# motionlife/gqmap-opticalflow

Measured on AMD Instinct MI355X. Metric: Gpixel-iters/s + AEPE vs .flo GT, Middlebury 584x388, 1/2/4/8 GPU, higher is better.
Workload: dtype f64; 1 GPU; C2: rubberwhale 584x388 mixture L=1 K=9 its=2541 (one step = one full-frame iteration); engine=mixture, L=1, K=9, parallelism=frame-parallel x1

## Files before the change

gqmap-opticalflow_amd/csrc/gqmap_engine.hip:

```cpp
#include <dlfcn.h>
#include <hip/hip_runtime.h>
#include <rccl/rccl.h>

#include <algorithm>
#include <chrono>
#include <condition_variable>
#include <cstdlib>
#include <cmath>
#include <cstring>
#include <mutex>
#include <string>
#include <vector>

#include "gqmap_internal.h"
#include "gqmap_blockmatch.h"

#pragma clang fp contract(off)

namespace gq {
__device__ __forceinline__ double gq_sqrt_dev(double x)
{
    const double y = __builtin_amdgcn_rsq(x);
    double g = x * y, h = 0.5 * y;
    const double r = fma(-h, g, 0.5);
// ... 67 lines not shown
    }
    __device__ __forceinline__ float end() const { return rp > 0.f ? sp : r; }
};
}
#define GQ_ROOT_STAGED 1

#define GQ_HD __device__ __forceinline__
#define GQ_SQRT(x) gq::gq_sqrt_dev(x)
#include "gqmap_tuning.h"
#define GQ_STR2(x) #x
#define GQ_PRAGMA_UNROLL(n) _Pragma(GQ_STR2(unroll n))
#define GQ_UNROLL2 GQ_PRAGMA_UNROLL(GQ_EDGE_UNROLL_N)
#define GQ_PAIR_UNROLL GQ_PRAGMA_UNROLL(GQ_PAIR_UNROLL_N)
#define GQ_PAIR_UNROLL_K(n) GQ_PRAGMA_UNROLL(n)
#define GQ_NODE_UNROLL GQ_PRAGMA_UNROLL(GQ_NODE_UNROLL_N)
#define GQ_UNROLL_FULL _Pragma("unroll")
#define GQ_UMUL24(a, b) __umul24((uint32_t)(a), (uint32_t)(b))
#define GQ_FRACT(x) __builtin_amdgcn_fract(x)
#define GQ_LDS_AS __attribute__((address_space(3)))
#define GQ_LUT_AT(lut, o) (*(const GQ_LDS_AS double *)((const GQ_LDS_AS char *)(lut) + (o)))
#define GQ_SCHED_FENCE __builtin_amdgcn_sched_barrier(0)
#define GQ_PIN64(x) asm volatile("" : "+v"(x))
#define GQ_PIN_UNIFORM(x) asm volatile("" : "+s"(x))
#include "gqmap_math.h"

namespace gq {

typedef float vvs_t;

constexpr int TILE = 16;
constexpr int BLOCK = TILE * TILE;
constexpr int TS = TAB_STRIDE;
constexpr int NPLANES = 9;
constexpr int TRACE_CAP = 8192;
constexpr int GRAPH_CHUNK = 50;
#ifndef GQ_FLOW_CHUNK
#define GQ_FLOW_CHUNK 250
#endif
constexpr int FLOW_CHUNK = GQ_FLOW_CHUNK;
static_assert(FLOW_CHUNK >= 1 && FLOW_CHUNK <= TRACE_CAP, "a launch's trace rows fit the ring");
constexpr int NFIX = 5;
constexpr int ACC_SLICES = 8;
constexpr int TRACE_W = 4;

struct Ctl {
    int it;
    int done;
    int stop;
    int arrive;
    double T;
    double alpha[GQMAP_LMAX];
    double w[GQMAP_LMAX];
    unsigned long long acc[ACC_SLICES][NFIX + GQMAP_LMAX][4];
    alignas(128) int it_i;
    int done_i;
    double T_i;
// ... 49 lines not shown
};

template <typename R>
using ctab_t = const __attribute__((address_space(4))) R *;
template <typename R>
__device__ __forceinline__ ctab_t<R> as_const(const R *p)
{
    return (ctab_t<R>)p;
}

__device__ __forceinline__ fix128 shfl_xor_fix(fix128 v, int o)
{
    const int64_t hi = (int64_t)(v >> 64);
    const uint64_t lo = (uint64_t)v;
    const int64_t h2 = __shfl_xor(hi, o, 64);
    const uint64_t l2 = (uint64_t)__shfl_xor((int64_t)lo, o, 64);
    return ((fix128)h2 << 64) | (fix128)l2;
}
__device__ __forceinline__ fix128 wave_sum_fix(fix128 v)
{
#pragma unroll
    for (int o = 32; o > 0; o >>= 1) v += shfl_xor_fix(v, o);
    return v;
}
__device__ __forceinline__ int wave_sum_small(int v)
{
    int s = 0;
#pragma unroll
    for (int b = 0; b < 6; ++b) s += __popcll(__ballot((v >> b) & 1)) << b;
    return s;
}
__device__ __forceinline__ bool finite_d(double x) { return (bits_of(x) & 0x7ff0000000000000ULL) != 0x7ff0000000000000ULL; }

__device__ __forceinline__ double shfl_xor_r(double v, int o) { return __shfl_xor(v, o, 64); }
__device__ __forceinline__ float shfl_xor_r(float v, int o) { return __shfl_xor(v, o, 64); }

typedef float f2v __attribute__((ext_vector_type(2)));

__device__ __forceinline__ f2v pk_fma(f2v a, f2v b, f2v c) { return __builtin_elementwise_fma(a, b, c); }

__device__ __forceinline__ f2v sqrt2_pk(f2v x)
{
    const f2v s = {__builtin_amdgcn_sqrtf(x.x), __builtin_amdgcn_sqrtf(x.y)};
    const f2v sm = {__int_as_float(__float_as_int(s.x) - 1), __int_as_float(__float_as_int(s.y) - 1)};
    const f2v sp = {__int_as_float(__float_as_int(s.x) + 1), __int_as_float(__float_as_int(s.y) + 1)};
    const f2v rm = pk_fma(-sm, s, x), rp = pk_fma(-sp, s, x);
// ... 296 lines not shown
           nn + P.n_off <= P.Ng - 2;
}

template <bool COH, typename R>
__device__ __forceinline__ R ld_state(const R *p)
{
    if constexpr (COH) return __hip_atomic_load(p, __ATOMIC_RELAXED, __HIP_MEMORY_SCOPE_AGENT);
    else return *p;
}
template <bool COH, typename R, bool NT = false>
__device__ __forceinline__ void st_state(R *p, R v)
{
    if constexpr (COH) __hip_atomic_store(p, v, __ATOMIC_RELAXED, __HIP_MEMORY_SCOPE_AGENT);
    else if constexpr (NT) __builtin_nontemporal_store(v, p);
    else *p = v;
}

template <typename R>
struct EdgeJob {
    int dir, uv, hr;
    bool need;
    R u1, o1, p, o2, u2;
};
template <typename R, typename VT, int Q, int TM, int TN, bool COH>
__device__ __forceinline__ EdgeJob<R> edge_job(const IterParams<R, VT> &P, const R *__restrict__ src, int e,
                                               int tid, int m, int n, int m0, int n0, int64_t loff, bool inner,
                                               bool valid, R mu_u, R mu_v, R sg_u, R sg_v)
{
    EdgeJob<R> jb{};
    int hm, hn, rm, rn;
    const bool own_edge = e < 4;
    if (own_edge) {
        jb.dir = e & 1; jb.uv = e >> 1;
        hm = m; hn = n;
        rm = jb.dir == 0 ? m + 1 : m; rn = jb.dir == 1 ? n + 1 : n;
    } else {
        const int h = tid / Q;
        const bool top = h < 2 * TN;
        const int hh = top ? h : h - 2 * TN, span = top ? TN : TM;
        jb.uv = hh / span;
        jb.hr = hh % span;
        jb.dir = top ? 0 : 1;
        hm = top ? m0 - 1 : m0 + jb.hr; hn = top ? n0 + jb.hr : n0 - 1;
        rm = top ? m0 : hm;             rn = top ? hn : n0;
    }
    const int M = P.M, N = P.N;
    const int64_t MNL = P.MNL;
    const bool r_inner = rm < M && rn < N && node_interior(P, rm, rn);
    jb.need = own_edge ? (inner || (valid && r_inner)) : (hm >= 0 && hn >= 0 && r_inner);
    if (jb.need) {
        const int uv = jb.uv;
        const int64_t h = hm + (int64_t)M * hn + loff;
        const int64_t r = rm + (int64_t)M * rn + loff;
        jb.u1 = own_edge ? (uv ? mu_v : mu_u) : ld_state<COH>(src + h + MNL * uv);
        jb.o1 = own_edge ? (uv ? sg_v : sg_u) : ld_state<COH>(src + h + MNL * (2 + uv));
        jb.p = ld_state<COH>(src + h + MNL * (5 + jb.dir + 2 * uv));
        jb.o2 = ld_state<COH>(src + r + MNL * (2 + uv));
        jb.u2 = ld_state<COH>(src + r + MNL * uv);
    }
    return jb;
}

#ifndef GQ_FLOW_TL
#define GQ_FLOW_TL 0
#endif

template <typename R>
struct HaloChain {
    R s[6][64];
    unsigned flag[4];
    unsigned *fail;
};
// ... 100 lines not shown
    __shared__ unsigned long long sh[4 * (NFIX + GQMAP_LMAX)];
    if (tid < 4 * NP) {
        unsigned long long *a = &ctl->acc[0][0][0] + tid;
        unsigned long long v[ACC_SLICES];
#pragma unroll
        for (int x = 0; x < ACC_SLICES; ++x) v[x] = __hip_atomic_load(a + x * SL, __ATOMIC_RELAXED, __HIP_MEMORY_SCOPE_AGENT);
        unsigned long long t = 0;
#pragma unroll
        for (int x = 0; x < ACC_SLICES; ++x) t += v[x];
#pragma unroll
        for (int x = 0; x < ACC_SLICES; ++x) __hip_atomic_store(a + x * SL, 0ull, __ATOMIC_RELAXED, __HIP_MEMORY_SCOPE_AGENT);
        sh[tid] = t;
    }
    __syncthreads();
    if (tid < NP) {
        fix128 v = 0;
#pragma unroll
        for (int k = 3; k >= 0; --k) v = (v << 32) + (fix128)(long long)sh[4 * tid + k];
        out[tid] = v;
    }
    if (tid == 0) ctl->arrive = 0;
}

template <typename R, typename VT>
__device__ __forceinline__ auto tile_frame_view(const IterParams<R, VT> &P, const GQ_LDS_AS double *taplut)
{
    if constexpr (is_vvo2<VT>::value) {
        return frame_view_lut(P.VV, P.M2, taplut);
    } else {
        (void)taplut;
        return frame_view(P.VV, P.M2);
    }
}

template <typename R, typename VT, int ENG, int Q, bool EDGE_FIRST, bool COH = false, bool NT = false,
          bool LIT = false, bool GRP = false, int ROTF = GQ_NODE_ROT_OTHER, int HALO = 0>
__device__ __forceinline__ void iter_tile(const IterParams<R, VT> P, int tile, int it, int parity,
                                          int part_r, TileLdsQ<R, Q> &lds, int l0, int l1, double Tcur,
                                          bool tab_ready, unsigned long long *acc_ring = nullptr,
                                          int grows = 0, bool grouped = false, HaloChain<R> *hc = nullptr,
                                          unsigned halo_tok = 0, const GQ_LDS_AS double *taplut = nullptr
#if GQ_FLOW_TL
                                          , unsigned long long *tlw = nullptr
#endif
                                          )
{
    static_assert(HALO == 0 || (GRP && sizeof(R) == 8), "the halo forms: the fp64 dataflow item (one component per item)");
    constexpr bool CHAIN = HALO == 1;
    static_assert(!LIT || (ENG == 0 && Q == 1 && sizeof(R) == 8), "literal order: fp64 mixture, Q = 1");
    static_assert(!GRP || (Q == 1 && !LIT), "a tile per wave: one lane per node");
    constexpr bool RS = Q == 0;
    constexpr int QA = arith_q(Q);
    constexpr int TPIX = tile_pix(Q);
    constexpr int TM = tile_rows(Q), TN = TPIX / TM;
    static_assert(TM * TN == TPIX, "tile");
    Ctl *ctl = P.ctl;
    const R *__restrict__ src = parity ? P.st1 : P.st0;
    R *__restrict__ dst = parity ? P.st0 : P.st1;
    const R T = R(Tcur);
    const R step = R(P.step0 / (1.0 + it / P.step_decay));

    const int tm = tile % P.tiles_m, tn = tile / P.tiles_m;
    const int tid = threadIdx.x;
    const int rtid = RS ? tid % TPIX : tid;
    const bool do_node = !RS || tid < TPIX, do_edge = !RS || tid >= TPIX;
    const int pix = rtid / QA, kj = rtid % QA;
    int lm = pix % TM, ln = pix / TM;
    if constexpr (GRP) {
        lm = (tid & 63) % grows;
        ln = (grouped ? 0 : (tid >> 6) * (64 / TM)) + (tid & 63) / grows;
    }
// ... 43 lines not shown
        const int64_t i = m + (int64_t)M * n + MN * l;
        const R mu_u = valid ? ld_state<COH>(src + i) : R(0);
        const R mu_v = valid ? ld_state<COH>(src + i + MNL) : R(0);
        const R sg_u = valid ? ld_state<COH>(src + i + MNL * 2) : R(0);
        const R sg_v = valid ? ld_state<COH>(src + i + MNL * 3) : R(0);
        const R pn = valid ? ld_state<COH>(src + i + MNL * 4) : R(0);
        Grad<R> nd{};
        R sum_mu0 = 0, sum_mu1 = 0, sum_sg0 = 0, sum_sg1 = 0;
        R eE = 0, eda = 0;
#pragma unroll
        for (int ph = 0; ph < 2; ++ph) {
        if ((ph == 0) != EDGE_FIRST) {
        if (do_node && LIT) {
            if constexpr (LIT)
                if (inner)
                    nd = lit_node_grad(tab, K2, P.VV, P.M2, P.I1, P.Mo, P.No, P.epsn, P.lamd, P.guard != 0, T, a,
                                       mu_u, mu_v, sg_u, sg_v, pn, m, n + P.n_off);
        } else if (do_node) {
        NodeCoef<R> c{};
        if (inner) c = node_coef(sg_u, sg_v, pn);
        const bool fast = ENG == 0 && __all(!inner || node_unclamped(c, mu_u, mu_v, m, n + P.n_off, P.Mo, P.No,
                                                                     P.gh_xmax, R(ENG == 2 ? CTF_MARGIN : 0.0)));
        if (inner) {
            const auto fv = tile_frame_view(P, taplut);
            constexpr bool PF = QA >= GQ_NODE_PF_MIN_Q && (QA > 1 || sizeof(VT) == 4);
            constexpr int ROT = PF ? ROTF : 0;
            Sums<R> S = fast ? node_sums<ENG, false, PF, ROT>(tab, kj, K2, QA, fv, P.I1, P.Mo, P.No, P.epsn, c, mu_u,
                                                              mu_v, m, n + P.n_off)
                             : node_sums<ENG, true, PF, ROT>(tab, kj, K2, QA, fv, P.I1, P.Mo, P.No, P.epsn, c, mu_u,
                                                             mu_v, m, n + P.n_off);
            if (QA > 1) S = lane_combine<QA>(S);
            nd = node_epi(S, c, P.lamd, P.guard != 0, T, a, sg_u, sg_v, pn, ENG == 2);
            if constexpr (RS) {
                lds.nd[0][pix] = nd.du1; lds.nd[1][pix] = nd.du2; lds.nd[2][pix] = nd.do1;
                lds.nd[3][pix] = nd.do2; lds.nd[4][pix] = nd.dp; lds.nd[5][pix] = nd.E; lds.nd[6][pix] = nd.da;
            }
        }
        }
        } else if (do_edge) {
        static_assert(HALO_LANES % QA == 0, "a node's lanes share their job count");
        const int njobs = halo_lane || chain ? 5 : 4;
        constexpr bool PREFETCH = QA >= GQ_PREFETCH_MIN_Q;
        auto job_at = [&](int e) {
            return edge_job<R, VT, QA, TM, TN, COH>(P, src, e, htid, m, n, m0, n0, MN * l, inner, valid, mu_u, mu_v,
                                                sg_u, sg_v);
        };
        EdgeJob<R> next{};
        if (PREFETCH) next = job_at(0);
        constexpr bool JOBS_UNROLLED = QA >= GQ_UNROLL_MIN_Q && ENG != 1;
        constexpr int JOB_UNROLL = JOBS_UNROLLED ? 5 : 1;
        static_assert(!CHAIN || (!PREFETCH && !JOBS_UNROLLED), "the chain: one job body, streamed");
#pragma unroll JOB_UNROLL
        for (int st = 0; st < (JOBS_UNROLLED ? 5 : njobs); ++st) {
            if (JOBS_UNROLLED && st >= njobs) continue;
            int e = st;
            bool slice = false, last = true;
            if constexpr (CHAIN)
                if (chain) {
                    slice = st == cw;
                    e = slice ? 4 : st - (st > cw);
                    last = !slice || cw == 3;
                }
            EdgeJob<R> jb;
            if (PREFETCH) {
                jb = next;
                if (st + 1 < njobs) next = job_at(st + 1);
            } else {
                jb = job_at(e);
// ... 34 lines not shown
                    g = edge_epi(S, c, P.lams, P.guard != 0, T, a, jb.o1, jb.o2, jb.p, ENG == 2);
                    }
                }
                if (own_edge && inner && lead)
                    st_state<COH, R, NT>(dst + i + MNL * (5 + e), fmin(fmax(jb.p + g.dp * step, -P.corr), P.corr));
            }
            if (own_edge) {
                if (uv == 0) { sum_mu0 = sum_mu0 + g.du1; sum_sg0 = sum_sg0 + g.do1; }
                else         { sum_mu1 = sum_mu1 + g.du1; sum_sg1 = sum_sg1 + g.do1; }
                eE = eE + g.E;
                eda = eda + g.da;
                if constexpr (GRP) {
                    if (dir == 0 && lm + 1 < grows && ln < TN) { in_up[uv][0][pix + 1] = g.du2; in_up[uv][1][pix + 1] = g.do2; }
                    if (dir == 1 && ln + 1 < TN) { in_left[uv][0][pix + grows] = g.du2; in_left[uv][1][pix + grows] = g.do2; }
                } else {
                if (lead && dir == 0 && lm + 1 < TM) { in_up[uv][0][pix + 1] = g.du2; in_up[uv][1][pix + 1] = g.do2; }
                if (lead && dir == 1 && ln + 1 < TN) { in_left[uv][0][pix + TM] = g.du2; in_left[uv][1][pix + TM] = g.do2; }
                }
            } else if constexpr (GRP) {
                const int hb = grouped ? wave * 64 : 0;
                if (CHAIN && !last) {
                    if constexpr (CHAIN) halo_chain_pass(hc, halo_tok, cw, lane, hs);
                } else
                if (dir == 0) { in_up[uv][0][hb + hr * grows] = g.du2; in_up[uv][1][hb + hr * grows] = g.do2; }
                else if (hr < grows) { in_left[uv][0][hb + hr] = g.du2; in_left[uv][1][hb + hr] = g.do2; }
            } else if (rtid % QA == 0) {
                if (dir == 0) { in_up[uv][0][hr * TM] = g.du2; in_up[uv][1][hr * TM] = g.do2; }
                else          { in_left[uv][0][hr] = g.du2; in_left[uv][1][hr] = g.do2; }
            }
#if GQ_FLOW_TL
            if (tlw && lane == 0 && own_edge) tlw[4 * cw + 1] = __builtin_amdgcn_s_memrealtime();
#endif
        }
        }
        if (ph == 0) TL_STAMP(1, __builtin_amdgcn_s_memrealtime());
        }
#if GQ_FLOW_TL
        if (tlw && lane == 0) {
            tlw[4 * cw] = (unsigned)__builtin_amdgcn_s_getreg((31 << 11) | 4);
            tlw[4 * cw + 2] = __builtin_amdgcn_s_memrealtime();
        }
#endif
        __syncthreads();
        TL_STAMP(2, __builtin_amdgcn_s_memrealtime());
        fix128 fda = 0;
        if (inner && lead && do_edge) {
            if constexpr (RS) {
                nd.du1 = lds.nd[0][pix]; nd.du2 = lds.nd[1][pix]; nd.do1 = lds.nd[2][pix];
                nd.do2 = lds.nd[3][pix]; nd.dp = lds.nd[4][pix]; nd.E = lds.nd[5][pix]; nd.da = lds.nd[6][pix];
            }
            const R gmu_u = ((nd.du1 + sum_mu0) + in_up[0][0][pix]) + in_left[0][0][pix];
            const R gmu_v = ((nd.du2 + sum_mu1) + in_up[1][0][pix]) + in_left[1][0][pix];
            const R gsg_u = ((nd.do1 + sum_sg0) + in_up[0][1][pix]) + in_left[0][1][pix];
            const R gsg_v = ((nd.do2 + sum_sg1) + in_up[1][1][pix]) + in_left[1][1][pix];
            fda = node_apply<ENG, COH, NT>(P, dst, i, m, n, step, mu_u, mu_v, sg_u, sg_v, pn, nd, gmu_u, gmu_v, gsg_u, gsg_v,
                                  eE, eda, fE, fmu, fsg, fae, nonfinite);
        }
        if (P.L > 1) {
            fda = wave_sum_fix(fda);
            if (lane == 0) red[NFIX + l][wave] = fda;
        }
        __syncthreads();
    }

    TL_STAMP(3, __builtin_amdgcn_s_memrealtime());
    fE = wave_sum_fix(fE);
    fmu = wave_sum_fix(fmu);
    fsg = wave_sum_fix(fsg);
    const fix128 fnf = (fix128)wave_sum_small(nonfinite);
    if (ENG == 2) fae = wave_sum_fix(fae);
    if (lane == 0) {
        red[0][wave] = fE;
        red[1][wave] = fmu;
        red[2][wave] = fsg;
        red[3][wave] = fnf;
        red[4][wave] = fae;
    }
    __syncthreads();
    const int NP = NFIX + P.L;
    if (tid < NP) {
        fix128 v = 0;
        const int lq = tid - NFIX;
        if (tid < NFIX || (P.L > 1 && lq >= l0 && lq < l1))
            v = (red[tid][0] + red[tid][1]) + (red[tid][2] + red[tid][3]);
        if (acc_ring) {
            if (v != 0) acc_add_agent(acc_ring + ((blockIdx.x % ACC_SLICES) * (NFIX + GQMAP_LMAX) + tid) * 4, v);
        } else if (P.fused || P.tile_acc) {
            if (v != 0) acc_add_agent(&ctl->acc[blockIdx.x % ACC_SLICES][tid][0], v);
        } else {
            store_part_agent(P.partials, P.fin.nblocks, part_r, tid, v);
        }
    }
}


template <typename R, typename VT, int ENG, int Q, bool NT = false, bool LIT = false>
__device__ __forceinline__ void k_iter_body(const IterParams<R, VT> &P)
{
    Ctl *ctl = P.ctl;
// ... 521 lines not shown
template <typename R, typename VT, int ENG, int Q, bool LIT = false, int W = 0>
__global__ __launch_bounds__(BLOCK, W > 0 ? W : LIT ? GQ_FLOW_LIT_WAVES : Q == 1 ? GQ_FLOW_WAVES : ENG == 1 ? 2 : min_waves(ENG, Q))
void k_iter_flow(IterParams<R, VT> P, int n_iter, unsigned *fl, int ntiles, const Ctl *snap)
{
    static_assert(Q >= 1 && Q <= 4, "1..4 lanes per node");
    static_assert(!LIT || (ENG == 0 && Q == 1), "literal order: the mixture engine at one lane per node");
    unsigned *bar = P.bar;
    const bool run = !snap->stop && __hip_atomic_load(&P.ctl->stop, __ATOMIC_RELAXED, __HIP_MEMORY_SCOPE_AGENT) == 0 &&
                     __hip_atomic_load(bar + BAR_FAIL, __ATOMIC_RELAXED, __HIP_MEMORY_SCOPE_AGENT) == 0;
    const int it0 = snap->it, done0 = snap->done;
    const double T0 = snap->T;
    const int b = blockIdx.x, xcd = b & 7;
    int s0 = 0;
    for (int y = 0; y < xcd; ++y) s0 += (ntiles - y + 7) >> 3;
    const int nb = (ntiles - xcd + 7) >> 3;
    const int L = ENG == 1 ? P.L : 1, nitems = ntiles * L;
    constexpr bool GRP = GQ_FLOW_GROUPS && Q == 1 && !LIT && (ENG == 0 || ENG == 2);
    constexpr int ROTF = ENG == 0 && Q == 1 && !LIT && W == 0 && sizeof(R) == 8 && is_vvpair<VT>::value
                             ? ((is_vvo2<VT>::value ? 0 : GQ_NODE_ROT_FLOW_FP64) | NODE_UNROLL(GQ_NODE_UNROLL_FLOW_FP64))
                             : GQ_NODE_ROT_OTHER;
    constexpr int HALO = !GRP || LIT || W != 0 || sizeof(R) != 8 ? 0
                         : ENG == 0 && is_vvpair<VT>::value ? GQ_FLOW_HALO
                         : ENG == 2 ? GQ_FLOW_HALO_CTF : 0;
    HaloChain<R> *hc = nullptr;
    if constexpr (HALO == 1) {
        __shared__ HaloChain<R> sh_halo;
        hc = &sh_halo;
        if (threadIdx.x < 4) sh_halo.flag[threadIdx.x] = 0;
        if (threadIdx.x == 0) sh_halo.fail = bar + BAR_FAIL;
    }
    const GQ_LDS_AS double *taplut = nullptr;
    if constexpr (is_vvo2<VT>::value) {
        __shared__ double sh_taplut[TAPLUT_N];
        const int *hdr = reinterpret_cast<const int *>(P.VV + vv_elems(P.Mo, P.No));
        const int vmin = hdr[0], vn = min(hdr[1], TAPLUT_N);
        for (int e = threadIdx.x; e < vn; e += BLOCK) sh_taplut[e] = taplut_entry(e, vmin);
        taplut = (const GQ_LDS_AS double *)sh_taplut;
    }
    const int vr = P.M - (P.tiles_m - 1) * tile_rows(Q);
    const bool groups = GRP && GQ_FLOW_ROWS && vr <= 4;
    const int nlast = groups ? (s0 + nb) / P.tiles_m - s0 / P.tiles_m : 0;
    const int nbl = groups ? nb - nlast + ((nlast + 3) >> 2) : nb * L;
    constexpr int INV = ENG == 2 && Q == 1 ? GQ_PHASE_MIX_CTF_Q1_INV : GQ_PHASE_MIX_OTHER_INV;
    constexpr bool MIX = GQ_FLOW_MIX && ENG == 0 && (!LIT || GQ_FLOW_LIT_MIX);
    const bool edge_first = MIX && ((((b >> 3) / P.cu_slots) & 1) != INV);
    __shared__ TileLdsQ<R, Q> lds;
// ... 43 lines not shown
        if (GQ_FLOW_LAG > 2 && threadIdx.x == 0)
            __hip_atomic_fetch_max(fl + FL_MAXJ, (unsigned)(j + 1), __ATOMIC_RELAXED, __HIP_MEMORY_SCOPE_AGENT);
#if GQ_FLOW_TL
        const unsigned long long tl_go = __builtin_amdgcn_s_memrealtime();
#endif
        double T = T0;
        if (P.fin.t_decay_every > 0) {
            const int e = P.fin.t_decay_every;
            const int nd = (it + e - 1) / e - (it0 + e - 1) / e;
            for (int q = 0; q < nd; ++q) T = fmax(T * P.fin.drate, P.fin.t_min);
        }
        unsigned long long *slot = acc + (size_t)(j % FL_SLOTS) * FL_ACC_SLOT;
        const int l0 = ENG == 1 ? l : 0, l1 = ENG == 1 ? l + 1 : 1;
        const int wtile = GRP ? __builtin_amdgcn_readfirstlane(grouped ? sh_grp[threadIdx.x >> 6] : tile) : tile;
        const int wrows = grouped ? vr : tile_rows(Q);
#if GQ_FLOW_TL
        const size_t tlwi = (size_t)j * nitems + (size_t)tile * L + l;
        unsigned long long *tlw = (tlwi + 1) * 16 <= (size_t)(4 * FLOW_TL_WORDS) && snap->it == 1 ? g_flow_tlw + tlwi * 16 : nullptr;
#define GQ_TLW_ARG , tlw
#else
#define GQ_TLW_ARG
#endif
        if (MIX && edge_first)
            iter_tile<R, VT, ENG, Q, true, GQ_FLOW_COH, false, LIT, GRP, ROTF, HALO>(P, wtile, it, parity, 0, lds, l0, l1, T, false, slot,
                                                                                wrows, grouped, hc, (unsigned)i + 1, taplut GQ_TLW_ARG);
        else
            iter_tile<R, VT, ENG, Q, false, GQ_FLOW_COH, false, LIT, GRP, ROTF, HALO>(P, wtile, it, parity, 0, lds, l0, l1, T, false, slot,
                                                                                 wrows, grouped, hc, (unsigned)i + 1, taplut GQ_TLW_ARG);
#undef GQ_TLW_ARG
        asm volatile("s_waitcnt vmcnt(0)" ::: "memory");
        __syncthreads();
#if GQ_FLOW_TL
        const size_t tli = (size_t)j * nitems + (size_t)tile * L + l;
        if (threadIdx.x == 0 && (tli + 1) * 4 <= (size_t)FLOW_TL_WORDS && snap->it == 1) {
            unsigned long long *w = g_flow_tl + tli * 4;
            w[0] = tl_claim;
            w[1] = tl_go;
            w[2] = __builtin_amdgcn_s_memrealtime();
            w[3] = ((unsigned long long)__builtin_amdgcn_s_getreg((31 << 11) | 20) << 32) |
                   (unsigned)__builtin_amdgcn_s_getreg((31 << 11) | 4);
        }
#endif
        if (GRP && grouped && threadIdx.x > 0 && (int)threadIdx.x < gsize)
            __hip_atomic_store(fl + FL_DONE + sh_grp[threadIdx.x], (unsigned)(j + 1), __ATOMIC_RELAXED, __HIP_MEMORY_SCOPE_AGENT);
        if (threadIdx.x == 0) {
            __hip_atomic_store(fl + FL_DONE + tile * L + l, (unsigned)(j + 1), __ATOMIC_RELAXED, __HIP_MEMORY_SCOPE_AGENT);
            const unsigned tk = __hip_atomic_fetch_add(fl + FL_ARR + (j % FL_SLOTS) * FL_LINE, (unsigned)gsize, __ATOMIC_RELAXED,
                                                       __HIP_MEMORY_SCOPE_AGENT);
            if (GQ_FLOW_PAIR) sh_i = (int)__hip_atomic_fetch_add(q, 1u, __ATOMIC_RELAXED, __HIP_MEMORY_SCOPE_AGENT);
            sh_last = tk == (unsigned)(nitems - gsize);
// ... 1248 lines not shown
    }
    if (c->lit) return false;
    if constexpr (sizeof(R) == 8) {
        switch (c->kq) {
        case 1: return launch_flow_q<R, VT, 2, 1>(c, n, dry);
        case 2: return launch_flow_q<R, VT, 2, 2>(c, n, dry);
        case 4: return c->pol.flow > 0 && launch_flow_q<R, VT, 2, 4>(c, n, dry);
        default: return false;
        }
    }
    return false;
}

bool launch_flow(gqmap_ctx *c, int n, bool dry)
{
    const bool on = c->pol.flow > 0 || (c->pol.flow < 0 && !c->fp32);
    if (!on || c->persist_off || (c->L != 1 && c->opt.engine != GQMAP_ENGINE_SUPER) || c->n_tiles != 1 ||
        c->comm || c->nranks != 0 || !fused_finalize(c) || n < 1)
        return false;
    if (c->fp32)
        return c->vvp ? !c->lit && c->kq == 1 && launch_flow_q<float, vvh2_t, 0, 1>(c, n, dry)
                      : launch_flow_t<float, float>(c, n, dry);
#if GQ_TAP_LUT
    if (c->vvp && c->tapt && c->tiles_m * c->tiles_n <= GQ_FLOW_WIDE_ITEMS)
        return !c->lit && c->kq == 1 && launch_flow_q<double, vvo2_t, 0, 1>(c, n, dry);
#endif
    if (c->vvp) return !c->lit && c->kq == 1 && launch_flow_q<double, vvh2_t, 0, 1>(c, n, dry);
    if (c->vv32) return launch_flow_t<double, vvs_t>(c, n, dry);
    return launch_flow_t<double, double>(c, n, dry);
}

gqmap_status persist_recover(gqmap_ctx *c, bool *recovered)
{
    *recovered = false;
    if (!c->d_snap) return GQMAP_OK;
    c->ctl_known = false;
    unsigned f = 0;
    GQ_HIP(hipMemcpyAsync(&f, c->d_bar + BAR_FAIL, sizeof(f), hipMemcpyDeviceToHost, c->stream));
    GQ_HIP(hipStreamSynchronize(c->stream));
    if (f == 0) return GQMAP_OK;
    Ctl h;
    GQ_HIP(hipMemcpyAsync(&h, c->d_snap_ctl, sizeof(Ctl), hipMemcpyDeviceToHost, c->stream));
    GQ_HIP(hipStreamSynchronize(c->stream));
    GQ_HIP(hipMemcpyAsync(c->d_st[h.done & 1], c->d_snap, c->snap_bytes, hipMemcpyDeviceToDevice, c->stream));
    GQ_HIP(hipMemcpyAsync(c->d_ctl, c->d_snap_ctl, sizeof(Ctl), hipMemcpyDeviceToDevice, c->stream));
    GQ_HIP(hipMemsetAsync(c->d_bar, 0, sizeof(unsigned) * BAR_WORDS, c->stream));
    if (c->d_flow) GQ_HIP(hipMemsetAsync(c->d_flow, 0, sizeof(unsigned) * c->flow_n, c->stream));
// ... 1498 lines not shown
```

gqmap-opticalflow_amd/csrc/gqmap_math.h:

```cpp
#pragma once
#include <stdint.h>
#include <string.h>

#include <type_traits>

namespace gq {

#ifndef GQ_M_PI
#define GQ_M_PI 3.14159265358979323846
#define GQ_M_SQRT2 1.41421356237309504880
#endif

constexpr int TAB_STRIDE = 256;
constexpr int NTAB = 8;
constexpr int T_XI = 0, T_XJ = 1, T_W = 2, T_WA = 3, T_WXI = 4, T_WXJ = 5, T_WM = 6, T_WX = 7;
#ifdef __HIPCC__
__host__ __device__
#endif
constexpr int tab_at(int r, int k) { return k * NTAB + r; }

GQ_HD uint64_t bits_of(double x)
{
    uint64_t u;
    memcpy(&u, &x, 8);
// ... 100 lines not shown
    w0 = fma(t2, R(2) - t, -t);
    w1 = fma(-t2, b, R(2) - t2);
    w2 = fma(t2, b, t);
    w3 = fma(t2, t, -t2);
}

#ifndef GQ_FRACT
#define GQ_FRACT(x) ((x) - floor(x))
#endif

#ifndef GQ_UMUL24
#define GQ_UMUL24(a, b) ((uint32_t)(a) * (uint32_t)(b))
#endif

template <typename VP>
GQ_HD VP byte_ptr(VP VV, uint32_t bytes)
{
    return (VP)((const char *)VV + bytes);
}
template <typename VP>
GQ_HD VP elem_ptr(VP VV, uint32_t elem)
{
    return byte_ptr(VV, elem * (uint32_t)sizeof(*VV));
}

#if defined(__HIPCC__)
struct alignas(4) vvh2_t {
    _Float16 lo, hi;
};
template <typename T>
struct is_vvh2 : std::is_same<typename std::remove_cv<T>::type, vvh2_t> {};
#else
template <typename T>
struct is_vvh2 : std::false_type {};
#endif
constexpr int TAPLUT_N = 1276;
struct alignas(4) vvo2_t {
    uint16_t lo, hi;
};
template <typename T>
struct is_vvo2 : std::is_same<typename std::remove_cv<T>::type, vvo2_t> {};
template <typename T>
struct is_vvpair : std::integral_constant<bool, is_vvh2<T>::value || is_vvo2<T>::value> {};
#ifdef __HIPCC__
__host__ __device__
#endif
// ... 136 lines not shown

template <typename VP>
struct TapView {
    VP p;
    uint32_t ld;
    GQ_HD uint32_t cell(int iy, int ix) const { return cell_elem(iy, ix, (int)ld); }
};
template <typename VP>
GQ_HD TapView<VP> frame_view(VP VV, int M2)
{
    return TapView<VP>{VV, (uint32_t)M2};
}
template <typename VP, typename LP>
struct TapViewLut {
    VP p;
    uint32_t ld;
    LP lut;
    GQ_HD uint32_t cell(int iy, int ix) const { return cell_elem(iy, ix, (int)ld); }
};
template <typename VP, typename LP>
GQ_HD TapViewLut<VP, LP> frame_view_lut(VP VV, int M2, LP lut)
{
    return TapViewLut<VP, LP>{VV, (uint32_t)M2, lut};
}
template <typename LP>
GQ_HD Taps16<double> lut_taps16(LP lut, const Taps16<vvo2_t> &T, uint32_t mask = 0xffffu, uint32_t shift = 16)
{
    Taps16<double> D;
    for (int c = 0; c < 4; ++c)
        for (int r = 0; r < 4; ++r) {
            const vvo2_t &e = T.v[4 * (c >> 1) + r];
            const uint32_t w = (uint32_t)e.lo | (uint32_t)e.hi << 16;
            D.v[4 * c + r] = GQ_LUT_AT(lut, (c & 1) ? w >> shift : w & mask);
        }
    return D;
}

constexpr int VV_TAIL = 8;
constexpr size_t vv_elems(int Mo, int No) { return (size_t)(Mo + 2) * (size_t)(No + 3) + VV_TAIL; }

template <bool CLAMP = true>
GQ_HD void axis_cell_abs(double X, int n, int &ix, double &fr)
{
    if (CLAMP) X = fmin(fmax(X, 1.0), (double)n);
    ix = (int)X;
    fr = GQ_FRACT(X);
// ... 373 lines not shown

template <typename R>
struct NodeCoef {
    R s, t, ax, bx, ay, by;
};
template <typename R>
GQ_HD NodeCoef<R> node_coef(R o1, R o2, R p)
{
    NodeCoef<R> c;
    spectral_st(p, c.s, c.t);
    const R sq2 = R(GQ_M_SQRT2);
    c.ax = sq2 * o1 * c.s; c.bx = sq2 * o1 * c.t;
    c.ay = sq2 * o2 * c.t; c.by = sq2 * o2 * c.s;
    return c;
}
constexpr int NODE_ROT = 1, NODE_ROT_STAGE = 2, NODE_ROT_FLAGS = 255;
constexpr int NODE_UNROLL(int n) { return n << 8; }
constexpr int node_rot_unroll(int rot) { return (rot >> 8) > 1 ? (rot >> 8) : 1; }
#ifndef GQ_SCHED_FENCE
#define GQ_SCHED_FENCE (void)0
#define GQ_PIN64(x) (void)(x)
#define GQ_PIN_UNIFORM(x) (void)(x)
#endif
template <bool CLAMP, int UNR, typename TP, typename TV, typename IP>
GQ_HD Sums<double> node_sums_lut(TP tab, int k0, int K2, int dk, const TV &V, IP I1, int Mo, int No, double eps,
                                 const NodeCoef<double> &c, double u1, double u2, int m, int n)
{
    Sums<double> S;
    if (k0 >= K2) return S;
    const double I = I1[m + (int64_t)Mo * n];
    const double U1 = u1 + double(n + 1), U2 = u2 + double(m + 1);
    auto locate = [&](double xi, double xj, double &so, double &to) -> uint32_t {
        const double x1 = fma(c.ax, xi, fma(c.bx, xj, U1));
        const double x2 = fma(c.ay, xi, fma(c.by, xj, U2));
        return cell4_abs_v<CLAMP>(V, Mo, No, x1, x2, so, to);
    };
    const int klast = k0 + (K2 - 1 - k0) / dk * dk;
    double so, to;
    auto T = load_taps16(V.p, locate(tab[tab_at(T_XI, k0)], tab[tab_at(T_XJ, k0)], so, to), V.ld);
    const int kn0 = k0 + dk <= klast ? k0 + dk : klast;
    double nxi = tab[tab_at(T_XI, kn0)], nxj = tab[tab_at(T_XJ, kn0)];
    auto trip = [&](int k) {
        uint32_t mask = 0xffffu, shift = 16;
        GQ_PIN_UNIFORM(mask);
        GQ_PIN_UNIFORM(shift);
        const Taps16<double> D = lut_taps16(V.lut, T, mask, shift);
        GQ_SCHED_FENCE;
        double sok = so, tok = to;
        T = load_taps16(V.p, locate(nxi, nxj, so, to), V.ld);
        GQ_SCHED_FENCE;
        GQ_PIN64(sok);
        GQ_PIN64(tok);
        const int kn2 = k + 2 * dk <= klast ? k + 2 * dk : klast;
        nxi = tab[tab_at(T_XI, kn2)];
        nxj = tab[tab_at(T_XJ, kn2)];
        const double d = fma(bicubic_taps4<double>(D, sok, tok), -0.25, I);
        S.add(tab, k, GQ_SQRT(fma(d, d, eps)));
        GQ_PIN64(S.s0); GQ_PIN64(S.sxi); GQ_PIN64(S.sxj);
        GQ_PIN64(S.sa); GQ_PIN64(S.sm); GQ_PIN64(S.sx);
        GQ_SCHED_FENCE;
    };
    int k = k0;
    GQ_PAIR_UNROLL_K(1)
    for (; k + (UNR - 1) * dk <= klast; k += UNR * dk) {
        GQ_UNROLL_FULL
        for (int u = 0; u < UNR; ++u) trip(k + u * dk);
    }
    if constexpr (UNR > 1) {
        GQ_PAIR_UNROLL_K(1)
        for (; k <= klast; k += dk) trip(k);
    }
    return S;
}
template <int ENG, bool CLAMP = true, bool PF = false, int ROT = 0, typename R, typename TP, typename TV, typename IP>
GQ_HD Sums<R> node_sums(TP tab, int k0, int K2, int dk, const TV &V, IP I1, int Mo, int No,
                        R eps, const NodeCoef<R> &c, R u1, R u2, int m, int n)
{
    Sums<R> S;
    if constexpr (is_vvo2<typename std::remove_cv<typename std::remove_reference<decltype(*V.p)>::type>::type>::value) {
// ... 504 lines not shown
```

gqmap-opticalflow_amd/csrc/gqmap_tuning.h:

```cpp
#pragma once

#ifndef GQ_EDGE_UNROLL_N
#define GQ_EDGE_UNROLL_N 2
#endif
#ifndef GQ_PAIR_UNROLL_N
#define GQ_PAIR_UNROLL_N 2
#endif
#ifndef GQ_PAIR_UNROLL_Q1
#define GQ_PAIR_UNROLL_Q1 4
#endif
#ifndef GQ_NODE_UNROLL_N
#define GQ_NODE_UNROLL_N 1
#endif
#ifndef GQ_FIN_GROUP
#define GQ_FIN_GROUP 1
#endif
#ifndef GQ_EDGE_PK
#define GQ_EDGE_PK 1
#endif
#ifndef GQ_TAB_LDS
#define GQ_TAB_LDS 1
#endif
#ifndef GQ_PHASE_MIX
#define GQ_PHASE_MIX 1
// ... 26 lines not shown
#define GQ_NODE_ROT_FLOW_FP64 0
#endif
#ifndef GQ_NODE_ROT_OTHER
#define GQ_NODE_ROT_OTHER 0
#endif
#ifndef GQ_FLOW_HALO
#define GQ_FLOW_HALO 1
#endif
#ifndef GQ_FLOW_HALO_CTF
#define GQ_FLOW_HALO_CTF 1
#endif
#ifndef GQ_FLOW_HALO_ROT_WAVE
#define GQ_FLOW_HALO_ROT_WAVE 2
#endif
#ifndef GQ_FLOW_HALO_EPI
#define GQ_FLOW_HALO_EPI 8
#endif
#ifndef GQ_FLOW_HALO_SLEEP
#define GQ_FLOW_HALO_SLEEP 1
#endif
#ifndef GQ_TAP_LUT
#define GQ_TAP_LUT 1
#endif
#ifndef GQ_UNROLL_MIN_Q
#define GQ_UNROLL_MIN_Q 2
#endif
#ifndef GQ_PERSIST_Q4
#define GQ_PERSIST_Q4 0
#endif
#ifndef GQ_PERSIST_SLEEP
#define GQ_PERSIST_SLEEP 2
#endif
#ifndef GQ_TIMELINE
#define GQ_TIMELINE 0
#endif
```

Baseline: 1.865 Gpixel-iter/s.

## Trim fp64 mixture tile: biased tap addressing, 32-bit edge addresses, DPP fixed-point sums

Adds three switchable trims, all on by default, to the fp64 mixture per-wave item on the offset-packed frame store. Tap loads use a pre-biased base pointer and 24-bit multiplies so each 16-tap gather needs less address arithmetic. Edge-state loads use 32-bit umul24 offsets, guarded on the host by a size check. The three 128-bit fixed-point wave reductions use inline-asm DPP add-with-carry chains in place of shuffle loops. Each cuts integer/VALU overhead, at the cost of fragile hand-written asm and narrower addressing limits.

```diff
diff --git a/gqmap-opticalflow_amd/csrc/gqmap_engine.hip b/gqmap-opticalflow_amd/csrc/gqmap_engine.hip
--- a/gqmap-opticalflow_amd/csrc/gqmap_engine.hip
+++ b/gqmap-opticalflow_amd/csrc/gqmap_engine.hip
@@ -113,6 +113,9 @@
 #define GQ_SCHED_FENCE __builtin_amdgcn_sched_barrier(0)
 #define GQ_PIN64(x) asm volatile("" : "+v"(x))
 #define GQ_PIN_UNIFORM(x) asm volatile("" : "+s"(x))
+#define GQ_PIN_UNIFORM64(x) asm volatile("" : "+s"(x))
+#define GQ_GLOBAL_AS __attribute__((address_space(1)))
+#define GQ_FRAME_WORD_AT(addr) (*(const GQ_GLOBAL_AS uint32_t *)(addr))
 #include "gqmap_math.h"
 
 namespace gq {
@@ -123,6 +126,7 @@
 constexpr int BLOCK = TILE * TILE;
 constexpr int TS = TAB_STRIDE;
 constexpr int NPLANES = 9;
+static_assert(NPLANES == EDGE_ADDR_PLANES, "edge_addr32_ok bounds a buffer of NPLANES planes");
 constexpr int TRACE_CAP = 8192;
 constexpr int GRAPH_CHUNK = 50;
 #ifndef GQ_FLOW_CHUNK
@@ -218,6 +222,38 @@
 #pragma unroll
     for (int o = 32; o > 0; o >>= 1) v += shfl_xor_fix(v, o);
     return v;
+}
+__device__ __forceinline__ void wave_sum_fix3_dpp(fix128 &a, fix128 &b, fix128 &c)
+{
+    unsigned a0 = (unsigned)a, a1 = (unsigned)(a >> 32), a2 = (unsigned)(a >> 64), a3 = (unsigned)(a >> 96);
+    unsigned b0 = (unsigned)b, b1 = (unsigned)(b >> 32), b2 = (unsigned)(b >> 64), b3 = (unsigned)(b >> 96);
+    unsigned c0 = (unsigned)c, c1 = (unsigned)(c >> 32), c2 = (unsigned)(c >> 64), c3 = (unsigned)(c >> 96);
+#define GQ_DPP_ADD128(x0, x1, x2, x3, ctl)                         \
+    "v_add_co_u32_dpp " x0 ", vcc, " x0 ", " x0 " " ctl "\n"       \
+    "v_addc_co_u32_dpp " x1 ", vcc, " x1 ", " x1 ", vcc " ctl "\n" \
+    "v_addc_co_u32_dpp " x2 ", vcc, " x2 ", " x2 ", vcc " ctl "\n" \
+    "v_addc_co_u32_dpp " x3 ", vcc, " x3 ", " x3 ", vcc " ctl "\n"
+#define GQ_DPP_STEP(ctl)                                                                 \
+    GQ_DPP_ADD128("%0", "%1", "%2", "%3", ctl) GQ_DPP_ADD128("%4", "%5", "%6", "%7", ctl) \
+    GQ_DPP_ADD128("%8", "%9", "%10", "%11", ctl)
+    asm volatile("s_nop 4\n"
+                 GQ_DPP_STEP("row_shr:1 row_mask:0xf bank_mask:0xf bound_ctrl:0")
+                 GQ_DPP_STEP("row_shr:2 row_mask:0xf bank_mask:0xf bound_ctrl:0")
+                 GQ_DPP_STEP("row_shr:4 row_mask:0xf bank_mask:0xf bound_ctrl:0")
+                 GQ_DPP_STEP("row_shr:8 row_mask:0xf bank_mask:0xf bound_ctrl:0")
+                 GQ_DPP_STEP("row_bcast:15 row_mask:0xa bank_mask:0xf")
+                 GQ_DPP_STEP("row_bcast:31 row_mask:0xc bank_mask:0xf")
+                 "s_nop 1"
+                 : "+v"(a0), "+v"(a1), "+v"(a2), "+v"(a3), "+v"(b0), "+v"(b1), "+v"(b2), "+v"(b3), "+v"(c0), "+v"(c1),
+                   "+v"(c2), "+v"(c3)
+                 :
+                 : "vcc");
+#undef GQ_DPP_STEP
+#undef GQ_DPP_ADD128
+    typedef unsigned __int128 u128;
+    a = (fix128)(((u128)a3 << 96) | ((u128)a2 << 64) | ((u128)a1 << 32) | a0);
+    b = (fix128)(((u128)b3 << 96) | ((u128)b2 << 64) | ((u128)b1 << 32) | b0);
+    c = (fix128)(((u128)c3 << 96) | ((u128)c2 << 64) | ((u128)c1 << 32) | c0);
 }
 __device__ __forceinline__ int wave_sum_small(int v)
 {
@@ -560,7 +596,7 @@
     bool need;
     R u1, o1, p, o2, u2;
 };
-template <typename R, typename VT, int Q, int TM, int TN, bool COH>
+template <typename R, typename VT, int Q, int TM, int TN, bool COH, bool A32 = false>
 __device__ __forceinline__ EdgeJob<R> edge_job(const IterParams<R, VT> &P, const R *__restrict__ src, int e,
                                                int tid, int m, int n, int m0, int n0, int64_t loff, bool inner,
                                                bool valid, R mu_u, R mu_v, R sg_u, R sg_v)
@@ -586,6 +622,21 @@
     const int64_t MNL = P.MNL;
     const bool r_inner = rm < M && rn < N && node_interior(P, rm, rn);
     jb.need = own_edge ? (inner || (valid && r_inner)) : (hm >= 0 && hn >= 0 && r_inner);
+    if constexpr (A32) {
+      if (jb.need) {
+        const uint32_t uv = (uint32_t)jb.uv, mnl = (uint32_t)MNL;
+        const uint32_t h = edge_elem32(hm, hn, M, (uint32_t)loff);
+        const uint32_t r = edge_elem32(rm, rn, M, (uint32_t)loff);
+        auto at = [&](uint32_t node, uint32_t plane) {
+            return (const R *)((const char *)src + (edge_plane_elem32(node, plane, mnl) * (uint32_t)sizeof(R)));
+        };
+        jb.u1 = own_edge ? (uv ? mu_v : mu_u) : ld_state<COH>(at(h, uv));
+        jb.o1 = own_edge ? (uv ? sg_v : sg_u) : ld_state<COH>(at(h, 2 + uv));
+        jb.p = ld_state<COH>(at(h, 5 + (uint32_t)jb.dir + 2 * uv));
+        jb.o2 = ld_state<COH>(at(r, 2 + uv));
+        jb.u2 = ld_state<COH>(at(r, uv));
+      }
+    } else
     if (jb.need) {
         const int uv = jb.uv;
         const int64_t h = hm + (int64_t)M * hn + loff;
@@ -732,10 +783,12 @@
     if (tid == 0) ctl->arrive = 0;
 }
 
-template <typename R, typename VT>
+template <bool BIAS = false, typename R, typename VT>
 __device__ __forceinline__ auto tile_frame_view(const IterParams<R, VT> &P, const GQ_LDS_AS double *taplut)
 {
-    if constexpr (is_vvo2<VT>::value) {
+    if constexpr (is_vvo2<VT>::value && BIAS) {
+        return frame_view_lut_biased(P.VV, P.M2, taplut);
+    } else if constexpr (is_vvo2<VT>::value) {
         return frame_view_lut(P.VV, P.M2, taplut);
     } else {
         (void)taplut;
@@ -743,8 +796,9 @@
     }
 }
 
+constexpr int TRIM_TAP_BIAS = 1, TRIM_EDGE_ADDR32 = 2, TRIM_FIXSUM_DPP = 4;
 template <typename R, typename VT, int ENG, int Q, bool EDGE_FIRST, bool COH = false, bool NT = false,
-          bool LIT = false, bool GRP = false, int ROTF = GQ_NODE_ROT_OTHER, int HALO = 0>
+          bool LIT = false, bool GRP = false, int ROTF = GQ_NODE_ROT_OTHER, int HALO = 0, int TRIM = 0>
 __device__ __forceinline__ void iter_tile(const IterParams<R, VT> P, int tile, int it, int parity,
                                           int part_r, TileLdsQ<R, Q> &lds, int l0, int l1, double Tcur,
                                           bool tab_ready, unsigned long long *acc_ring = nullptr,
@@ -757,6 +811,7 @@
 {
     static_assert(HALO == 0 || (GRP && sizeof(R) == 8), "the halo forms: the fp64 dataflow item (one component per item)");
     constexpr bool CHAIN = HALO == 1;
+    static_assert(TRIM == 0 || (GRP && ENG == 0 && is_vvo2<VT>::value), "the trimmed item: the fp64 mixture item on the offset store");
     static_assert(!LIT || (ENG == 0 && Q == 1 && sizeof(R) == 8), "literal order: fp64 mixture, Q = 1");
     static_assert(!GRP || (Q == 1 && !LIT), "a tile per wave: one lane per node");
     constexpr bool RS = Q == 0;
@@ -846,7 +901,7 @@
         const bool fast = ENG == 0 && __all(!inner || node_unclamped(c, mu_u, mu_v, m, n + P.n_off, P.Mo, P.No,
                                                                      P.gh_xmax, R(ENG == 2 ? CTF_MARGIN : 0.0)));
         if (inner) {
-            const auto fv = tile_frame_view(P, taplut);
+            const auto fv = tile_frame_view<(TRIM & TRIM_TAP_BIAS) != 0>(P, taplut);
             constexpr bool PF = QA >= GQ_NODE_PF_MIN_Q && (QA > 1 || sizeof(VT) == 4);
             constexpr int ROT = PF ? ROTF : 0;
             Sums<R> S = fast ? node_sums<ENG, false, PF, ROT>(tab, kj, K2, QA, fv, P.I1, P.Mo, P.No, P.epsn, c, mu_u,
@@ -866,8 +921,8 @@
         const int njobs = halo_lane || chain ? 5 : 4;
         constexpr bool PREFETCH = QA >= GQ_PREFETCH_MIN_Q;
         auto job_at = [&](int e) {
-            return edge_job<R, VT, QA, TM, TN, COH>(P, src, e, htid, m, n, m0, n0, MN * l, inner, valid, mu_u, mu_v,
-                                                sg_u, sg_v);
+            return edge_job<R, VT, QA, TM, TN, COH, (TRIM & TRIM_EDGE_ADDR32) != 0>(P, src, e, htid, m, n, m0, n0, MN * l, inner,
+                                                                                    valid, mu_u, mu_v, sg_u, sg_v);
         };
         EdgeJob<R> next{};
         if (PREFETCH) next = job_at(0);
@@ -948,7 +1003,14 @@
                 if (CHAIN && !last) {
                     if constexpr (CHAIN) halo_chain_pass(hc, halo_tok, cw, lane, hs);
                 } else
-                if (dir == 0) { in_up[uv][0][hb + hr * grows] = g.du2; in_up[uv][1][hb + hr * grows] = g.do2; }
+                if (dir == 0) {
+                    if constexpr ((TRIM & TRIM_EDGE_ADDR32) != 0) {
+                        const int hrg = (int)__umul24((unsigned)hr, (unsigned)grows);
+                        in_up[uv][0][hb + hrg] = g.du2; in_up[uv][1][hb + hrg] = g.do2;
+                    } else {
+                        in_up[uv][0][hb + hr * grows] = g.du2; in_up[uv][1][hb + hr * grows] = g.do2;
+                    }
+                }
                 else if (hr < grows) { in_left[uv][0][hb + hr] = g.du2; in_left[uv][1][hb + hr] = g.do2; }
             } else if (rtid % QA == 0) {
                 if (dir == 0) { in_up[uv][0][hr * TM] = g.du2; in_up[uv][1][hr * TM] = g.do2; }
@@ -990,6 +1052,17 @@
     }
 
     TL_STAMP(3, __builtin_amdgcn_s_memrealtime());
+    if constexpr ((TRIM & TRIM_FIXSUM_DPP) != 0) {
+        wave_sum_fix3_dpp(fE, fmu, fsg);
+        const fix128 fnf = (fix128)wave_sum_small(nonfinite);
+        if (lane == 63) {
+            red[0][wave] = fE;
+            red[1][wave] = fmu;
+            red[2][wave] = fsg;
+            red[3][wave] = fnf;
+            red[4][wave] = fae;
+        }
+    } else {
     fE = wave_sum_fix(fE);
     fmu = wave_sum_fix(fmu);
     fsg = wave_sum_fix(fsg);
@@ -1001,6 +1074,7 @@
         red[2][wave] = fsg;
         red[3][wave] = fnf;
         red[4][wave] = fae;
+    }
     }
     __syncthreads();
     const int NP = NFIX + P.L;
@@ -1568,6 +1642,10 @@
     constexpr int HALO = !GRP || LIT || W != 0 || sizeof(R) != 8 ? 0
                          : ENG == 0 && is_vvpair<VT>::value ? GQ_FLOW_HALO
                          : ENG == 2 ? GQ_FLOW_HALO_CTF : 0;
+    constexpr int TRIM = ENG == 0 && Q == 1 && !LIT && W == 0 && sizeof(R) == 8 && GRP && is_vvo2<VT>::value
+                             ? (GQ_TAP_BIAS ? TRIM_TAP_BIAS : 0) | (GQ_EDGE_ADDR32 ? TRIM_EDGE_ADDR32 : 0) |
+                                   (GQ_FIXSUM_DPP ? TRIM_FIXSUM_DPP : 0)
+                             : 0;
     HaloChain<R> *hc = nullptr;
     if constexpr (HALO == 1) {
         __shared__ HaloChain<R> sh_halo;
@@ -1657,10 +1735,10 @@
 #define GQ_TLW_ARG
 #endif
         if (MIX && edge_first)
-            iter_tile<R, VT, ENG, Q, true, GQ_FLOW_COH, false, LIT, GRP, ROTF, HALO>(P, wtile, it, parity, 0, lds, l0, l1, T, false, slot,
+            iter_tile<R, VT, ENG, Q, true, GQ_FLOW_COH, false, LIT, GRP, ROTF, HALO, TRIM>(P, wtile, it, parity, 0, lds, l0, l1, T, false, slot,
                                                                                 wrows, grouped, hc, (unsigned)i + 1, taplut GQ_TLW_ARG);
         else
-            iter_tile<R, VT, ENG, Q, false, GQ_FLOW_COH, false, LIT, GRP, ROTF, HALO>(P, wtile, it, parity, 0, lds, l0, l1, T, false, slot,
+            iter_tile<R, VT, ENG, Q, false, GQ_FLOW_COH, false, LIT, GRP, ROTF, HALO, TRIM>(P, wtile, it, parity, 0, lds, l0, l1, T, false, slot,
                                                                                  wrows, grouped, hc, (unsigned)i + 1, taplut GQ_TLW_ARG);
 #undef GQ_TLW_ARG
         asm volatile("s_waitcnt vmcnt(0)" ::: "memory");
@@ -2955,7 +3033,8 @@
         return c->vvp ? !c->lit && c->kq == 1 && launch_flow_q<float, vvh2_t, 0, 1>(c, n, dry)
                       : launch_flow_t<float, float>(c, n, dry);
 #if GQ_TAP_LUT
-    if (c->vvp && c->tapt && c->tiles_m * c->tiles_n <= GQ_FLOW_WIDE_ITEMS)
+    if (c->vvp && c->tapt && c->tiles_m * c->tiles_n <= GQ_FLOW_WIDE_ITEMS &&
+        (!GQ_EDGE_ADDR32 || edge_addr32_ok(c->M, c->N, c->L, sizeof(double))))
         return !c->lit && c->kq == 1 && launch_flow_q<double, vvo2_t, 0, 1>(c, n, dry);
 #endif
     if (c->vvp) return !c->lit && c->kq == 1 && launch_flow_q<double, vvh2_t, 0, 1>(c, n, dry);
diff --git a/gqmap-opticalflow_amd/csrc/gqmap_math.h b/gqmap-opticalflow_amd/csrc/gqmap_math.h
--- a/gqmap-opticalflow_amd/csrc/gqmap_math.h
+++ b/gqmap-opticalflow_amd/csrc/gqmap_math.h
@@ -146,6 +146,16 @@
 GQ_HD VP elem_ptr(VP VV, uint32_t elem)
 {
     return byte_ptr(VV, elem * (uint32_t)sizeof(*VV));
+}
+
+GQ_HD uint32_t edge_elem32(int m, int n, int M, uint32_t loff) { return (uint32_t)m + GQ_UMUL24(M, n) + loff; }
+GQ_HD uint32_t edge_plane_elem32(uint32_t node, uint32_t plane, uint32_t MNL) { return node + GQ_UMUL24(plane, MNL); }
+constexpr int EDGE_ADDR_PLANES = 9;
+constexpr bool edge_addr32_ok(int64_t M, int64_t N, int64_t L, int64_t elem_bytes)
+{
+    constexpr int64_t U24 = (int64_t)1 << 24, U32 = (int64_t)1 << 32;
+    return M >= 0 && N >= 0 && L >= 1 && M < U24 && N < U24 && M * N < U24 && M * N * L < U24 && M * N * L * L < U24 &&
+           EDGE_ADDR_PLANES * (M * N * L) * elem_bytes < U32;
 }
 
 #if defined(__HIPCC__)
@@ -328,6 +338,54 @@
 GQ_HD TapViewLut<VP, LP> frame_view_lut(VP VV, int M2, LP lut)
 {
     return TapViewLut<VP, LP>{VV, (uint32_t)M2, lut};
+}
+#ifndef GQ_FRAME_WORD_AT
+GQ_HD uint32_t frame_word_at(uintptr_t addr)
+{
+    uint32_t w;
+    memcpy(&w, (const void *)addr, sizeof w);
+    return w;
+}
+#define GQ_FRAME_WORD_AT(addr) frame_word_at(addr)
+#endif
+GQ_HD uint32_t tap_bias_elems(int M2) { return (uint32_t)M2 + 1u; }
+GQ_HD uint32_t cell_elem_biased(int iy, int ix, int M2) { return (uint32_t)iy + GQ_UMUL24(M2, ix); }
+template <typename VP, typename LP>
+struct TapViewLutBiased {
+    VP p;
+    uint32_t ld;
+    LP lut;
+    uintptr_t b0, b2;
+    GQ_HD uint32_t cell(int iy, int ix) const { return cell_elem_biased(iy, ix, (int)ld); }
+};
+template <typename VP, typename LP>
+GQ_HD TapViewLutBiased<VP, LP> frame_view_lut_biased(VP VV, int M2, LP lut)
+{
+    constexpr uintptr_t EB = sizeof(*VV);
+    const uintptr_t b0 = (uintptr_t)VV - EB * tap_bias_elems(M2);
+    return TapViewLutBiased<VP, LP>{VV, (uint32_t)M2, lut, b0, b0 + EB * 2u * (uint32_t)M2};
+}
+template <typename T>
+struct is_tap_biased : std::false_type {};
+template <typename VP, typename LP>
+struct is_tap_biased<TapViewLutBiased<VP, LP>> : std::true_type {};
+template <typename TV>
+GQ_HD auto view_taps16(const TV &V, uint32_t o)
+{
+    if constexpr (is_tap_biased<TV>::value) {
+        using E = typename std::remove_cv<typename std::remove_reference<decltype(*V.p)>::type>::type;
+        static_assert(is_vvo2<E>::value && sizeof(E) == 4, "the biased view: the offset store, an element one word");
+        const uint32_t ob = o * 4u;
+        Taps16<E> T;
+        for (int pr = 0; pr < 2; ++pr)
+            for (int r = 0; r < 4; ++r) {
+                const uint32_t w = GQ_FRAME_WORD_AT((pr ? V.b2 : V.b0) + ob + (uint32_t)(4 * r));
+                T.v[4 * pr + r] = E{(uint16_t)(w & 0xffffu), (uint16_t)(w >> 16)};
+            }
+        return T;
+    } else {
+        return load_taps16(V.p, o, V.ld);
+    }
 }
 template <typename LP>
 GQ_HD Taps16<double> lut_taps16(LP lut, const Taps16<vvo2_t> &T, uint32_t mask = 0xffffu, uint32_t shift = 16)
@@ -747,6 +805,9 @@
 #define GQ_PIN64(x) (void)(x)
 #define GQ_PIN_UNIFORM(x) (void)(x)
 #endif
+#ifndef GQ_PIN_UNIFORM64
+#define GQ_PIN_UNIFORM64(x) (void)(x)
+#endif
 template <bool CLAMP, int UNR, typename TP, typename TV, typename IP>
 GQ_HD Sums<double> node_sums_lut(TP tab, int k0, int K2, int dk, const TV &V, IP I1, int Mo, int No, double eps,
                                  const NodeCoef<double> &c, double u1, double u2, int m, int n)
@@ -762,7 +823,9 @@
     };
     const int klast = k0 + (K2 - 1 - k0) / dk * dk;
     double so, to;
-    auto T = load_taps16(V.p, locate(tab[tab_at(T_XI, k0)], tab[tab_at(T_XJ, k0)], so, to), V.ld);
+    auto T = view_taps16(V, locate(tab[tab_at(T_XI, k0)], tab[tab_at(T_XJ, k0)], so, to));
+    double mq = -0.25;
+    if constexpr (is_tap_biased<TV>::value) GQ_PIN_UNIFORM64(mq);
     const int kn0 = k0 + dk <= klast ? k0 + dk : klast;
     double nxi = tab[tab_at(T_XI, kn0)], nxj = tab[tab_at(T_XJ, kn0)];
     auto trip = [&](int k) {
@@ -772,14 +835,14 @@
         const Taps16<double> D = lut_taps16(V.lut, T, mask, shift);
         GQ_SCHED_FENCE;
         double sok = so, tok = to;
-        T = load_taps16(V.p, locate(nxi, nxj, so, to), V.ld);
+        T = view_taps16(V, locate(nxi, nxj, so, to));
         GQ_SCHED_FENCE;
         GQ_PIN64(sok);
         GQ_PIN64(tok);
         const int kn2 = k + 2 * dk <= klast ? k + 2 * dk : klast;
         nxi = tab[tab_at(T_XI, kn2)];
         nxj = tab[tab_at(T_XJ, kn2)];
-        const double d = fma(bicubic_taps4<double>(D, sok, tok), -0.25, I);
+        const double d = fma(bicubic_taps4<double>(D, sok, tok), mq, I);
         S.add(tab, k, GQ_SQRT(fma(d, d, eps)));
         GQ_PIN64(S.s0); GQ_PIN64(S.sxi); GQ_PIN64(S.sxj);
         GQ_PIN64(S.sa); GQ_PIN64(S.sm); GQ_PIN64(S.sx);
diff --git a/gqmap-opticalflow_amd/csrc/gqmap_tuning.h b/gqmap-opticalflow_amd/csrc/gqmap_tuning.h
--- a/gqmap-opticalflow_amd/csrc/gqmap_tuning.h
+++ b/gqmap-opticalflow_amd/csrc/gqmap_tuning.h
@@ -72,6 +72,15 @@
 #ifndef GQ_TAP_LUT
 #define GQ_TAP_LUT 1
 #endif
+#ifndef GQ_TAP_BIAS
+#define GQ_TAP_BIAS 1
+#endif
+#ifndef GQ_EDGE_ADDR32
+#define GQ_EDGE_ADDR32 1
+#endif
+#ifndef GQ_FIXSUM_DPP
+#define GQ_FIXSUM_DPP 1
+#endif
 #ifndef GQ_UNROLL_MIN_Q
 #define GQ_UNROLL_MIN_Q 2
 #endif
```

Result: faster. 1.902 Gpixel-iter/s, median of 6 (+2.0%).
